# vision-agh/apse_uav

Measured on AMD Instinct MI355X. Metric: 4K UAV frames/sec (whole node), higher is better.
Workload: dtype f32

## Files before the change

### apse_uav_amd/_lib.py

```python
import ctypes as C
import os

import numpy as np

_HERE = os.path.dirname(os.path.abspath(__file__))
_TREE_LIB = os.path.join(_HERE, "libapse_hip.so")
LIB_PATH = os.environ.get("APSE_HIP_LIB") or _TREE_LIB
TOOL_ENTRIES = ("apse_conv2d_ex", "apse_winograd_pack_filter", "apse_winograd_conv2d", "apse_winograd_conv2d_split", "apse_lane_stats", "apse_rpn_select", "apse_box_inference",
                "apse_c4_rpn_select", "apse_rpn_select_train", "apse_rpn_train_proposals_workspace_bytes", "apse_rpn_train_proposals",
                "apse_set_rpn_head", "apse_preprocess_frames_yuv", "apse_yuv_to_bgr", "apse_yuv_matrix_host", "apse_resize_normalize_yuv")

APSE_OK = 0


class ApseError(RuntimeError):
    pass


class Config(C.Structure):
    _fields_ = [
        ("struct_size", C.c_int), ("device", C.c_int), ("max_batch", C.c_int),
        ("frame_h", C.c_int), ("frame_w", C.c_int), ("image_h", C.c_int), ("image_w", C.c_int),
        ("blocks", C.c_int * 4), ("num_classes", C.c_int),
        ("score_thresh", C.c_float), ("box_nms", C.c_float), ("rpn_nms", C.c_float), ("mask_thresh", C.c_float),
        ("rpn_pre_topk", C.c_int), ("rpn_post_topk", C.c_int), ("dets_per_image", C.c_int),
        ("pixel_mean", C.c_float * 3), ("assoc_roi", C.c_int), ("embed_dim", C.c_int), ("assoc_scale", C.c_float),
        ("compute_dtype", C.c_int), ("storage16", C.c_int),
    ]


class ConfigArch(Config):
    _fields_ = [("arch", C.c_int)]


class ConfigLane(ConfigArch):
    _fields_ = [("tail_lane", C.c_int)]


class ResultsLayout(C.Structure):
    _fields_ = [("bytes", C.c_size_t), ("n_max", C.c_int), ("dets_per_image", C.c_int), ("embed_dim", C.c_int),
                ("max_batch", C.c_int)] + [(k, C.c_size_t) for k in (
# ... 30 lines not shown
    "apse_set_resize_tables": ([vp, vp, vp, i, vp, vp, i], i),
    "apse_set_camera": ([vp, C.POINTER(C.c_double), C.POINTER(C.c_double), i, vp, i, i], i),
    "apse_preprocess_frames": ([vp, vp, i, vp], i),
    "apse_preprocess_images": ([vp, vp, i, vp], i),
    "apse_backbone": ([vp, i, vp], i),
    "apse_rpn": ([vp, i, vp], i),
    "apse_rpn_levels": ([vp, i, i, vp], i),
    "apse_box_head": ([vp, i, vp], i),
    "apse_set_detections": ([vp, vp, vp, vp, vp, i, vp], i),
    "apse_mask_tail": ([vp, i, vp], i),
    "apse_embed": ([vp, i, vp], i),
    "apse_forward": ([vp, i, vp], i),
    "apse_results_describe": ([vp, C.POINTER(ResultsLayout)], i),
    "apse_read_results": ([vp, vp, sz, vp], i),
    "apse_read_results_begin": ([vp, vp, sz, vp], i),
    "apse_read_results_end": ([vp, vp], i),
    "apse_lane_stats": ([vp, C.POINTER(C.c_longlong * 4)], i),
    "apse_copy_mask_window": ([vp, i, i, i, i, i, vp, vp], i),
    "apse_copy_mask_windows": ([vp, i, vp, vp, vp, vp, vp], i),
    "apse_host_copy": ([vp, vp, sz, i], i),
    "apse_feature_shape": ([vp, C.c_char_p, C.POINTER(C.c_int * 3)], i),
    "apse_export_feature": ([vp, C.c_char_p, vp, i, vp], i),
    "apse_debug_tensor": ([vp, C.c_char_p, vp, sz, C.POINTER(sz), vp], i),
    "apse_flops": ([vp, i, C.c_double, C.c_double], C.c_double),
    "apse_profile": ([vp, i], i),
    "apse_profile_read": ([vp, C.POINTER(C.c_double * 42), i], i),
    "apse_conv_packed_elems": ([C.POINTER(ConvDesc)], sz),
    "apse_conv_pack_weight": ([C.POINTER(ConvDesc), vp, i, vp, vp], i),
    "apse_conv2d": ([C.POINTER(ConvDesc), vp, vp, vp, vp, vp, vp, sz, vp], i),
    "apse_conv2d_ex": ([C.POINTER(ConvDesc), vp, vp, vp, vp, vp, vp, sz, vp, i, i, i, vp], i),
    "apse_winograd_pack_filter": ([vp, i, i, vp], i),
    "apse_winograd_conv2d": ([C.POINTER(ConvDesc), vp, vp, vp, vp, vp], i),
    "apse_winograd_conv2d_split": ([C.POINTER(ConvDesc), vp, vp, vp, vp, vp, C.c_size_t, i, vp], i),
    "apse_maxpool3x3s2": ([vp, vp, i, i, i, i, vp], i),
    "apse_maxpool3x3s2_typed": ([vp, vp, i, i, i, i, i, vp], i),
    "apse_roi_align": ([C.POINTER(vp), C.POINTER(i), C.POINTER(i), vp, i, i, i, vp, vp], i),
    "apse_roi_align_typed": ([C.POINTER(vp), C.POINTER(i), C.POINTER(i), vp, i, i, i, i, vp, vp], i),
    "apse_roi_pool": ([vp, i, i, vp, vp, i, i, f, vp, vp], i),
    "apse_roi_features": ([vp, i, vp, vp, i, i, vp, vp], i),
    "apse_nms_rank": ([vp, vp, vp, i, i, i, i, f, i, vp, vp, vp, vp, vp], i),
    "apse_rpn_select": ([C.POINTER(vp), C.POINTER(i), C.POINTER(i), i, i, i, i, i, i, f, i, vp, vp, vp, vp, vp, vp, vp, vp, vp], i),
    "apse_box_inference": ([vp, i, i, vp, vp, i, i, i, i, f, f, i, i] + [vp] * 16, i),
    "apse_c4_rpn_select": ([vp, i, i, i, i, i, i, i, f, vp, vp, vp, vp, vp, vp, vp, vp], i),
    "apse_mask_centroid_dense": ([vp, i, i, C.POINTER(C.c_int * 3), vp], i),
    "apse_mask_closest_dense": ([vp, i, i, f, f, C.POINTER(C.c_int * 2), vp], i),
    "apse_l2_normalize": ([vp, vp, i, i, vp], i),
    "apse_sqdist": ([vp, vp, i, i, i, vp, vp], i),
    "apse_undistort_gamma": ([vp, vp, i, i, i, C.POINTER(C.c_double), C.POINTER(C.c_double), i, vp, i, i, vp], i),
    "apse_lab_tables_host": ([vp, vp, C.c_size_t], C.c_size_t),
    "apse_replay_create": ([i, i, f, i], vp),
    "apse_replay_destroy": ([vp], None),
    "apse_replay_step": ([vp, i, i, vp, vp, vp, C.c_char_p, i, vp], i),
    "apse_replay_packed": ([vp, vp, C.c_longlong, i, i, i, vp, C.c_longlong], C.c_longlong),
    "apse_replay_max_id": ([vp], i),
    "apse_replay_next_id": ([vp], i),
    "apse_render_workspace_bytes": ([i, i, i], sz),
    "apse_render_instances": ([vp, vp, i, i, i, i, vp, i, vp, sz, vp, i, vp, sz, vp], i),
    "apse_render_pack_mask": ([vp, i, i, vp, vp], i),
    "apse_render_font_host": ([vp, sz], sz),
    "apse_mots_split_workspace_bytes": ([], sz),
    "apse_mots_split_idmap": ([vp, i, i, i, vp, sz, vp, vp, vp, vp, sz, vp], i),
    "apse_mots_rle_to_bits": ([vp, vp, i, i, i, vp, vp], i),
    "apse_mots_overlaps": ([vp, i, vp, i, vp, i, vp, vp], i),
    "apse_mots_shift_overlaps": ([vp, i, vp, i, i, i, vp, vp], i),
    "apse_mots_render_idmap": ([vp, vp, i, i, i, vp, vp], i),
    "apse_mots_crop_overlaps": ([vp, vp, i, i, i, vp, sz, vp, vp, vp], i),
# ... 106 lines not shown
```

### apse_uav_amd/csrc/conv_igemm.hip

```cpp
#include "apse_common.h"
#include <type_traits>

typedef _Float16 f16x8 __attribute__((ext_vector_type(8)));
__device__ __forceinline__ f32x16 apse_mfma16(bf16x8 a, bf16x8 b, f32x16 c) { return __builtin_amdgcn_mfma_f32_32x32x16_bf16(a, b, c, 0, 0, 0); }
__device__ __forceinline__ f32x16 apse_mfma16(f16x8 a, f16x8 b, f32x16 c) { return __builtin_amdgcn_mfma_f32_32x32x16_f16(a, b, c, 0, 0, 0); }

template <int WM, int WN, int TM, int TN, int KS, int XT, int WK, int PR = 0>
__global__ __launch_bounds__(64 * WM * WN * WK) void conv_igemm_f32(const ConvParams p) {
    static_assert(PR == 0 || XT == 0, "16-bit operands use the descriptor path only");
    constexpr bool DESC = XT != 1;
    constexpr int EPS = PR ? 64 : 32;
    constexpr int ESH = PR ? 1 : 2;
    constexpr int EPSLOT = 16 >> ESH;
    constexpr int NT = 64 * WM * WN * WK;
    constexpr int BM = WM * TM * 32;
    constexpr int BN = WN * TN * 32;
    constexpr int SR = NT / 8;
    constexpr int AP = BM / SR;
    constexpr int BP = BN / SR;
    static_assert(AP >= 1 && BP >= 1 && KS % WK == 0 && (DESC || WK == 1), "unsupported shape");
    constexpr int LDC = BN + 4;
    constexpr bool DP = DESC && (TM * TN <= 2 || (PR != 0 && WM * WN == 8 && APSE_DP16));
    constexpr int NSET = DP ? 2 : 1;
    constexpr int STORE_AT = 4 * KS - 2;
    extern __shared__ __attribute__((aligned(16))) char smem[];
    float* As = reinterpret_cast<float*>(smem);
    float* Bs = As + 2 * KS * BM * 32;
    float* Cs = reinterpret_cast<float*>(smem);

    const int tid = threadIdx.x;
    const int lane = tid & 63;
    const int wave = tid >> 6;
    const int kg = wave / (WM * WN);
    const int wm = (wave % (WM * WN)) / WN, wn = wave % WN;
    const int fr = lane & 31, fh = lane >> 5;
    const int srow = tid >> 3, slot = tid & 7;

    int M = p.M;
    if (p.m_count) {
        int lim = (*p.m_count) * p.m_per_item;
        M = lim < M ? lim : M;
    }
    const int tiles_n = (p.Cout + BN - 1) / BN;
    const int tiles_m = (M + BM - 1) / BM;
    const int nwg = tiles_m * tiles_n;
    const int z = blockIdx.y;
    const int steps_per_row = p.KWCp / EPS;
    const int steps_total = PR ? p.KH * steps_per_row : p.steps_total;
    const int steps_big = (steps_total + KS - 1) / KS;
    const int per = (steps_big + p.splitk - 1) / p.splitk;
    const int s_begin = z * per;
    const int s_end = (s_begin + per < steps_big) ? s_begin + per : steps_big;
    const int ohw = p.OH * p.OW;
    const size_t w_row = (size_t)p.KH * p.KWCp;
    const bool direct = (p.splitk == 1);
    __amdgpu_buffer_rsrc_t xrsrc;
    if constexpr (DESC)
        xrsrc = __builtin_amdgcn_make_buffer_rsrc(const_cast<float*>(p.x), 0, (int)((((unsigned)(p.B * p.H * p.W) << p.cin_log2)) << (XT >= 2 ? 1 : ESH)), 0x00020000);

    bool warm_pending = p.next_w && z == 0;
    for (int wg = blockIdx.x; wg < nwg; wg += gridDim.x) {
        const int bid = apse_xcd_remap(wg, nwg);
        const int tile_m = bid / tiles_n, tile_n = bid - tile_m * tiles_n;
        const int m0 = tile_m * BM, n0 = tile_n * BN;

        int a_iy0[AP], a_ix0[AP], a_pix[AP], a_base[AP];
#pragma unroll
        for (int i = 0; i < AP; ++i) {
            const int m = m0 + srow + SR * i;
            if (m < M) {
                const int b = m / ohw;
                const int rem = m - b * ohw;
                const int oy = rem / p.OW;
                const int ox = rem - oy * p.OW;
                a_iy0[i] = oy * p.stride - p.pad;
                a_ix0[i] = ox * p.stride - p.pad;
                a_pix[i] = b * p.H * p.W;
            } else {
                a_iy0[i] = -(1 << 28);
                a_ix0[i] = 0;
                a_pix[i] = 0;
            }
            a_base[i] = (a_pix[i] + a_iy0[i] * p.W + a_ix0[i]) << p.cin_log2;
        }

        f32x4 ra[NSET][KS][AP], rb[NSET][KS][BP];
        int ld_r, ld_q;
        {
            const int ss0 = s_begin * KS;
            ld_r = ss0 / steps_per_row;
            ld_q = ss0 - ld_r * steps_per_row;
        }
        const char* wrow[BP];
#pragma unroll
        for (int i = 0; i < BP; ++i)
            wrow[i] = (PR ? reinterpret_cast<const char*>(p.w16) : reinterpret_cast<const char*>(p.w)) +
                      ((((size_t)(n0 + srow + SR * i) * w_row) + (size_t)(slot * EPSLOT)) << ESH);
        int cur_r = 0, cur_ry = 0, cur_q = 0, cur_rowoff = 0, cur_woff = 0, cur_dpx = 0;
        auto fetch_piece = [&](int set, int u, int j) {
            if (j == 0) {
                const bool live = ld_r < p.KH;
                cur_r = live ? ld_r : p.KH - 1;
                cur_ry = live ? ld_r : (1 << 28);
                cur_q = ld_q * EPS + slot * EPSLOT;
                cur_dpx = cur_q >> p.cin_log2;
                cur_rowoff = ((cur_r * p.W) << p.cin_log2) + cur_q;
                cur_woff = (cur_r * p.KWCp + ld_q * EPS) << ESH;
                ++ld_q;
                if (ld_q == steps_per_row) { ld_q = 0; ++ld_r; }
            }
            if (j < AP) {
                const int iy = a_iy0[j] + cur_ry;
                const int px = a_ix0[j] + cur_dpx;
                const int okm = -(int)(((unsigned)iy < (unsigned)p.H) & ((unsigned)px < (unsigned)p.W));
                if constexpr (XT >= 2) {
                    const unsigned off = (((unsigned)(a_base[j] + cur_rowoff) << 1) & (unsigned)okm) | (0xfffffff0u & ~(unsigned)okm);
                    const auto raw = __builtin_amdgcn_raw_buffer_load_b64(xrsrc, (int)off, 0, 0);
                    ra[set][u][j] = f32x4{__uint_as_float(raw[0]), __uint_as_float(raw[1]), 0.f, 0.f};
                } else {
                    const unsigned off = (((unsigned)(a_base[j] + cur_rowoff) << ESH) & (unsigned)okm) | (0xfffffff0u & ~(unsigned)okm);
                    ra[set][u][j] = __builtin_bit_cast(f32x4, __builtin_amdgcn_raw_buffer_load_b128(xrsrc, (int)off, 0, 0));
                }
            } else {
                rb[set][u][j - AP] = *reinterpret_cast<const f32x4*>(wrow[j - AP] + cur_woff);
            }
        };
        auto store_piece = [&](int set, int buf, int u, int j) {
            if (j < AP) {
                const int row = srow + SR * j;
                const int ps = slot ^ ((row >> 1) & 7);
                f32x4 v = ra[set][u][j];
                if constexpr (XT == 2) {
// ... 472 lines not shown
            if (p.res_st == 1) return __uint_as_float((uint32_t)reinterpret_cast<const uint16_t*>(p.res)[idx] << 16);
            return (float)reinterpret_cast<const _Float16*>(p.res)[idx];
        };
        size_t dst;
        if (p.out_mode == 0) {
            if (p.res_mode == 1) {
                val += ld1((size_t)m * p.Cout + n);
            } else if (p.res_mode == 2) {
                const int b = m / ohw;
                const int rem = m - b * ohw;
                const int oy = rem / p.OW, ox = rem - oy * p.OW;
                const int hw2 = (p.OH >> 1) * (p.OW >> 1);
                val += ld1(((size_t)b * hw2 + (oy >> 1) * (p.OW >> 1) + (ox >> 1)) * p.Cout + n);
            }
            dst = (size_t)m * p.y_ld + p.y_coff + n;
        } else {
            const int b = m / ohw;
            const int rem = m - b * ohw;
            const int oy = rem / p.OW, ox = rem - oy * p.OW;
            const int dy = g >> 1, dx = g & 1;
            dst = (((size_t)b * 2 * p.OH + 2 * oy + dy) * (2 * p.OW) + 2 * ox + dx) * p.cdec + co;
        }
        if (p.relu) val = apse_relu(val);
        apse_st1(p.y, dst, val, p.y_st);
    }
}

void apse_launch_splitk_reduce4(const ConvParams& p, hipStream_t s) {
    int blocks = (int)(((size_t)p.M * p.Cout / 4 + 255) / 256);
    if (blocks > 4096) blocks = 4096;
    hipLaunchKernelGGL(conv_splitk_reduce4, dim3(blocks), dim3(256), 0, s, p);
}

template <int WM, int WN, int TM, int TN, int KS, int XT, int WK = 1, int PR = 0>
static int launch_cfg_x(const ConvParams& p, hipStream_t s, hipEvent_t ev0, hipEvent_t ev1) {
    constexpr int BM = WM * TM * 32, BN = WN * TN * 32;
    const int tiles = ((p.M + BM - 1) / BM) * ((p.Cout + BN - 1) / BN);
    const size_t lds_stage = (size_t)2 * KS * (BM + BN) * 32 * sizeof(float), lds_c = (size_t)WK * BM * (BN + 4) * sizeof(float) + 16;
    const size_t lds = lds_stage > lds_c ? lds_stage : lds_c;
    static bool attr_done = false;
    if (!attr_done) {
        hipFuncSetAttribute(reinterpret_cast<const void*>(&conv_igemm_f32<WM, WN, TM, TN, KS, XT, WK, PR>),
                            hipFuncAttributeMaxDynamicSharedMemorySize, (int)lds);
        attr_done = true;
    }
    int grid_x = tiles;
    if (p.m_count) {
        int want = 1024;
        if (p.m_hint > 0) {
            want = 2 * ((p.m_hint + BM - 1) / BM) * ((p.Cout + BN - 1) / BN);
            if (want < 64) want = 64;
            if (want > 1024) want = 1024;
        }
        if (grid_x > want) grid_x = want;
    }
    if (ev0) hipEventRecord(ev0, s);
    hipLaunchKernelGGL((conv_igemm_f32<WM, WN, TM, TN, KS, XT, WK, PR>), dim3(grid_x, p.splitk), dim3(64 * WM * WN * WK), lds, s, p);
    if (ev1) hipEventRecord(ev1, s);
    if (p.splitk > 1 && !p.tile_cnt) {
        const size_t total = (size_t)p.M * p.Cout;
        const bool vec4 = p.out_mode == 0 && (p.res_mode == 0 || p.res_mode == 1) && ((p.Cout | p.y_ld | p.y_coff) & 3) == 0 && total < 0x7fffffffull;
        int blocks = (int)(((vec4 ? total / 4 : total) + 255) / 256);
        if (blocks > 4096) blocks = 4096;
        if (vec4) hipLaunchKernelGGL(conv_splitk_reduce4, dim3(blocks), dim3(256), 0, s, p);
        else hipLaunchKernelGGL(conv_splitk_reduce, dim3(blocks), dim3(256), 0, s, p);
    }
    return hipGetLastError() == hipSuccess ? APSE_OK : APSE_E_HIP;
}

static bool descriptor_ok(const ConvParams& p) { return p.x_st == 0 && (((size_t)p.B * p.H * p.W) << p.cin_log2) * 4 < 0xfffffff0ull; }

template <int WM, int WN, int TM, int TN, int KS>
static int launch_cfg(const ConvParams& p, hipStream_t s, hipEvent_t ev0, hipEvent_t ev1) {
    return descriptor_ok(p) ? launch_cfg_x<WM, WN, TM, TN, KS, 0>(p, s, ev0, ev1) : launch_cfg_x<WM, WN, TM, TN, KS, 1>(p, s, ev0, ev1);
}
template <int WM, int WN, int TM, int TN, int KS, int KSF>
static int launch_cfg_k2(const ConvParams& p, hipStream_t s, hipEvent_t ev0, hipEvent_t ev1) {
    return descriptor_ok(p) ? launch_cfg_x<WM, WN, TM, TN, KS, 0, 2>(p, s, ev0, ev1) : launch_cfg_x<WM, WN, TM, TN, KSF, 1>(p, s, ev0, ev1);
}

static int fast16_shape(const ConvParams& p, int cfg) {
    const bool fast16 = (p.prec == 1 || p.prec == 2) && p.w16 && p.x_st == p.prec && (p.KWCp & 63) == 0 && p.cin_log2 >= 3 &&
                        ((((size_t)p.B * p.H * p.W) << p.cin_log2) * 2 < 0xfffffff0ull) && !p.tile_cnt;
    if (!fast16) return -1;
    int c16 = (cfg == 4 || cfg == 5 || cfg == 2) ? 1 : (cfg == 7 ? 6 : cfg);
    if (c16 == 0 && p.steps_total >= 16 && ((p.M + 255) / 256) * ((p.Cout + 127) / 128) >= 250) c16 = 8;
    return c16;
}

int apse_conv_effective_cfg(const ConvParams& p, int cfg) {
    if (cfg == APSE_CFG_STREAM) return (!p.no_stream && apse_conv1x1_stream_ok(p)) ? APSE_CFG_STREAM : -1;
    if (cfg == APSE_CFG_GLDS) return apse_conv_glds16_ok(p) ? APSE_CFG_GLDS : -1;
    if (cfg == APSE_CFG_SKINNY) return apse_conv_skinny_ok(p) ? APSE_CFG_SKINNY : -1;
    if (!p.no_stream && apse_conv_skinny_ok(p)) return APSE_CFG_SKINNY;
    if (!p.no_stream && apse_conv1x1_stream_ok(p)) return APSE_CFG_STREAM;
    if (!p.no_stream && apse_conv_glds16_ok(p)) {
        const int c16 = fast16_shape(p, cfg);
        if (c16 == 8) return APSE_CFG_GLDS;
        const int t128 = ((p.M + 127) / 128) * ((p.Cout + 127) / 128);
        if ((c16 == 0 || c16 == 3) && p.steps_total >= 16 && t128 >= 200 && t128 <= 320 && apse_conv_glds16_small(p)) return APSE_CFG_GLDS;
    }
    return cfg;
}

int apse_launch_conv(const ConvParams& p, int cfg, hipStream_t s, hipEvent_t ev0, hipEvent_t ev1) {
    if (p.M <= 0 || p.Cout <= 0 || p.steps_total <= 0) return APSE_E_INVALID;
    if (p.res_mode != 0 && (p.Cout & 3) != 0) return APSE_E_INVALID;
    const int eff = apse_conv_effective_cfg(p, cfg);
    if (eff < 0) return APSE_E_INVALID;
    if (eff == APSE_CFG_STREAM) return apse_launch_conv1x1_stream(p, s, ev0, ev1);
    if (eff == APSE_CFG_GLDS) return apse_launch_conv_glds16(p, s, ev0, ev1);
    if (eff == APSE_CFG_SKINNY) return apse_launch_conv_skinny(p, s, ev0, ev1);
    if (p.prec == 1 || p.prec == 2) {
        const int c16 = fast16_shape(p, cfg);
        if (c16 >= 0) {
            int rc = APSE_E_INVALID;
            if (p.prec == 1) {
                if (c16 == 0) rc = launch_cfg_x<2, 2, 2, 2, 1, 0, 1, 1>(p, s, ev0, ev1);
                else if (c16 == 1) rc = launch_cfg_x<2, 2, 1, 1, 2, 0, 1, 1>(p, s, ev0, ev1);
                else if (c16 == 3) rc = launch_cfg_x<4, 1, 1, 2, 1, 0, 1, 1>(p, s, ev0, ev1);
                else if (c16 == 6) rc = launch_cfg_x<2, 2, 1, 1, 2, 0, 2, 1>(p, s, ev0, ev1);
                else if (c16 == 8) rc = launch_cfg_x<4, 2, 2, 2, 1, 0, 1, 1>(p, s, ev0, ev1);
            } else {
                if (c16 == 0) rc = launch_cfg_x<2, 2, 2, 2, 1, 0, 1, 2>(p, s, ev0, ev1);
                else if (c16 == 1) rc = launch_cfg_x<2, 2, 1, 1, 2, 0, 1, 2>(p, s, ev0, ev1);
                else if (c16 == 3) rc = launch_cfg_x<4, 1, 1, 2, 1, 0, 1, 2>(p, s, ev0, ev1);
                else if (c16 == 6) rc = launch_cfg_x<2, 2, 1, 1, 2, 0, 2, 2>(p, s, ev0, ev1);
                else if (c16 == 8) rc = launch_cfg_x<4, 2, 2, 2, 1, 0, 1, 2>(p, s, ev0, ev1);
            }
            return rc;
        }
        return APSE_E_INVALID;
    }
    switch (cfg) {
        case 0: return launch_cfg<2, 2, 2, 2, 1>(p, s, ev0, ev1);
        case 1: return launch_cfg<2, 2, 1, 1, 2>(p, s, ev0, ev1);
        case 2: {
            const bool small = (((size_t)p.B * p.H * p.W) << p.cin_log2) * 4 < 0xfffffff0ull;
            if (small && p.x_st == 1 && p.cin_log2 >= 2) return launch_cfg_x<4, 1, 1, 1, 2, 2>(p, s, ev0, ev1);
            if (small && p.x_st == 2 && p.cin_log2 >= 2) return launch_cfg_x<4, 1, 1, 1, 2, 3>(p, s, ev0, ev1);
            return launch_cfg<4, 1, 1, 1, 2>(p, s, ev0, ev1);
        }
        case 3: return launch_cfg<4, 1, 1, 2, 1>(p, s, ev0, ev1);
        case 4: return launch_cfg<2, 2, 1, 1, 1>(p, s, ev0, ev1);
        case 5: return launch_cfg<4, 1, 1, 1, 1>(p, s, ev0, ev1);
        case 6: return launch_cfg_k2<2, 2, 1, 1, 2, 2>(p, s, ev0, ev1);
        case 7: return launch_cfg_k2<2, 2, 1, 1, 4, 2>(p, s, ev0, ev1);
        case 8: return launch_cfg<2, 2, 2, 2, 1>(p, s, ev0, ev1);
        default: return APSE_E_INVALID;
    }
}

int apse_conv_pick_cfg(int M, int Cout, int steps, int* splitk) {
    *splitk = 1;
    auto tiles = [&](int bm, int bn) { return ((M + bm - 1) / bm) * ((Cout + bn - 1) / bn); };
    auto split_for = [&](int t, int min_steps_per_split) {
        int sk = (512 + t / 2) / t;
        if (sk > steps / min_steps_per_split) sk = steps / min_steps_per_split;
        if (sk > 64) sk = 64;
        return sk < 1 ? 1 : sk;
    };
    if (Cout <= 32) {
        const int t = tiles(128, 32);
        if (t < 32 && steps >= 16) {
            int sk = 64 / t;
            if (sk > steps / 4) sk = steps / 4;
            if (sk > 8) sk = 8;
            *splitk = sk < 1 ? 1 : sk;
        }
        return 2;
    }
    if (Cout <= 64) return tiles(128, 64) >= 192 ? 3 : 1;
    const int t128 = tiles(128, 128);
    if (t128 >= 224) {
        if (t128 < 384 && tiles(128, 64) >= 384) return 3;
        return 0;
    }
    if (t128 >= 32 && steps >= 256) {
        *splitk = split_for(t128, 8);
// ... 15 lines not shown
```

### apse_uav_amd/csrc/conv_winograd.hip

```cpp
#include "apse_common.h"

namespace {
constexpr int WT = 64;
constexpr int WN = 64;
constexpr int KC = 8;
constexpr int NTHR = 512;
constexpr int G_U = 1, G_ROWS = 2, G_V = 3;
constexpr int SLICE_F = 16 * WT * KC;
constexpr size_t WINO_LDS = (size_t)2 * 2 * SLICE_F * sizeof(float);
static_assert(WN == WT, "V and U slices share one size");
static_assert((size_t)16 * WT * 32 * sizeof(float) <= WINO_LDS, "epilogue chunk must fit the staging LDS");
}

template <int WTR, int WTC, bool SPLIT>
__global__ __launch_bounds__(NTHR) void conv_winograd_f32(const ConvParams p) {
    static_assert(WTR * WTC == WT, "64 tiles per block");
    extern __shared__ __attribute__((aligned(16))) char smem[];
    float* Vs = reinterpret_cast<float*>(smem);
    float* Us = Vs + 2 * SLICE_F;
    float* Cs = reinterpret_cast<float*>(smem);

    const int tid = threadIdx.x;
    const int lane = tid & 63, wave = __builtin_amdgcn_readfirstlane(tid >> 6);
    const int fr = lane & 31, fh = lane >> 5;

    const int tiles_y = (p.OH + 2 * WTR - 1) / (2 * WTR), tiles_x = (p.OW + 2 * WTC - 1) / (2 * WTC);
    const int nblk = p.Cout / WN;
    const int nwg = p.B * tiles_y * tiles_x * nblk;
    const int bid = apse_xcd_remap(blockIdx.x, nwg);
    const int nb = bid % nblk;
    int rest = bid / nblk;
    const int bx = rest % tiles_x; rest /= tiles_x;
    const int by = rest % tiles_y;
// ... 11 lines not shown
    const int cg = tid & 1, t = (tid >> 1) & (WT - 1), ti = wave >> 1;
    const int ra = ti == 0 ? 0 : (ti == 2 ? 2 : 1);
    const int rb = ti == 0 ? 2 : (ti == 1 ? 2 : (ti == 2 ? 1 : 3));
    const float sgn = ti == 1 ? 1.f : -1.f;
    const int iy_a = oy0 + 2 * (t / WTC) - 1 + ra, iy_b = oy0 + 2 * (t / WTC) - 1 + rb;
    const int ix0 = ox0 + 2 * (t % WTC) - 1;
    const __amdgpu_buffer_rsrc_t xrsrc =
        __builtin_amdgcn_make_buffer_rsrc(const_cast<float*>(p.x), 0, (int)((((unsigned)(p.B * p.H * p.W)) << p.cin_log2) * 4u), 0x00020000);
    const __amdgpu_buffer_rsrc_t xnone = __builtin_amdgcn_make_buffer_rsrc(const_cast<float*>(p.x), 0, 0, 0x00020000);
    unsigned xoff[2][4];
#pragma unroll
    for (int r = 0; r < 2; ++r) {
        const int iy = r ? iy_b : iy_a;
#pragma unroll
        for (int c = 0; c < 4; ++c) {
            const int ix = ix0 + c;
            const bool in = (unsigned)iy < (unsigned)p.H && (unsigned)ix < (unsigned)p.W;
            xoff[r][c] = in ? ((((unsigned)((b * p.H + iy) * p.W + ix)) << p.cin_log2) + (unsigned)(cg * 4)) * 4u : 0x80000000u;
        }
    }
    const unsigned ustep = (unsigned)(16 * p.Cout * KC * 4);
    const __amdgpu_buffer_rsrc_t ursrc = __builtin_amdgcn_make_buffer_rsrc(
        const_cast<float*>(p.wu), 0, SPLIT ? (int)((unsigned)s_end * ustep) : (int)((((unsigned)(16 * p.Cout)) << p.cin_log2) * 4u), 0x00020000);
    unsigned uoff[4], ulds[4];
#pragma unroll
    for (int k = 0; k < 4; ++k) {
        const int q = tid + NTHR * k;
        const int xi = q >> 7, co = (q >> 1) & 63, h = q & 1;
        uoff[k] = (unsigned)(((xi * p.Cout + n0 + co) * KC + h * 4) * 4);
        ulds[k] = (unsigned)((xi * WN + co) * KC + ((h ^ ((co >> 3) & 1)) * 4));
    }
    const int vlds = (4 * ti * WT + t) * KC + (cg ^ ((t >> 3) & 1)) * 4;

    f32x4 xr[2][4], ur[4];
    auto fetch_u = [&](int s) {
        const unsigned kb = (unsigned)(s_begin + s) * ustep;
#pragma unroll
        for (int k = 0; k < 4; ++k) ur[k] = __builtin_bit_cast(f32x4, __builtin_amdgcn_raw_buffer_load_b128(ursrc, (int)(uoff[k] + kb), 0, 0));
    };
    auto fetch_x = [&](int s) {
        const unsigned kb = (unsigned)((s_begin + s) * KC * 4);
        const __amdgpu_buffer_rsrc_t rs = s < nsteps ? xrsrc : xnone;
#pragma unroll
        for (int r = 0; r < 2; ++r)
#pragma unroll
            for (int c = 0; c < 4; ++c)
                xr[r][c] = __builtin_bit_cast(f32x4, __builtin_amdgcn_raw_buffer_load_b128(rs, (int)(xoff[r][c] + kb), 0, 0));
    };
    auto write_u = [&](int buf) {
#pragma unroll
        for (int k = 0; k < 4; ++k) *reinterpret_cast<f32x4*>(Us + buf * SLICE_F + ulds[k]) = ur[k];
    };
    auto xform_rows = [&]() {
#pragma unroll
        for (int c = 0; c < 4; ++c)
#pragma unroll
            for (int e = 0; e < 4; ++e) xr[0][c][e] = __builtin_fmaf(xr[1][c][e], sgn, xr[0][c][e]);
    };
    auto write_v = [&](int buf) {
        const f32x4 v[4] = {xr[0][0] - xr[0][2], xr[0][1] + xr[0][2], xr[0][2] - xr[0][1], xr[0][1] - xr[0][3]};
#pragma unroll
        for (int j = 0; j < 4; ++j) *reinterpret_cast<f32x4*>(Vs + buf * SLICE_F + vlds + j * WT * KC) = v[j];
    };

    f32x16 acc[2][2][2];
#pragma unroll
    for (int a = 0; a < 2; ++a)
#pragma unroll
        for (int i = 0; i < 2; ++i)
#pragma unroll
            for (int j = 0; j < 2; ++j)
#pragma unroll
                for (int v = 0; v < 16; ++v) acc[a][i][j][v] = 0.f;

    fetch_u(0);
    fetch_x(0);
    write_u(0);
    xform_rows();
    write_v(0);
    __builtin_amdgcn_sched_barrier(0);
    fetch_u(1);
    __builtin_amdgcn_sched_barrier(0);
    fetch_x(1);
    __syncthreads();
    const int fsw = (fh ^ ((fr >> 3) & 1)) * 4;
    const int frag = (2 * wave * WT + fr) * KC + fsw;
    f32x4 af[2][2], bf[2][2];
    auto read_frags = [&](int buf, int a) {
#pragma unroll
        for (int i = 0; i < 2; ++i) af[a][i] = *reinterpret_cast<const f32x4*>(Vs + buf * SLICE_F + frag + (a * WT + 32 * i) * KC);
#pragma unroll
        for (int j = 0; j < 2; ++j) bf[a][j] = *reinterpret_cast<const f32x4*>(Us + buf * SLICE_F + frag + (a * WN + 32 * j) * KC);
    };
    auto mfma_group = [&](int a, int k) {
#pragma unroll
        for (int i = 0; i < 2; ++i)
#pragma unroll
            for (int j = 0; j < 2; ++j)
                acc[a][i][j] = __builtin_amdgcn_mfma_f32_32x32x2f32(af[a][i][k], bf[a][j][k], acc[a][i][j], 0, 0, 0);
    };
    read_frags(0, 0);
    for (int s = 0; s < nsteps; ++s) {
        const int buf = s & 1;
        read_frags(buf, 1);
#pragma unroll
        for (int g = 0; g < 7; ++g) {
            __builtin_amdgcn_sched_barrier(0);
            if (g == G_U) { write_u(buf ^ 1); fetch_u(s + 2); }
            if (g == G_ROWS) xform_rows();
            if (g == G_V) { write_v(buf ^ 1); fetch_x(s + 2); }
            __builtin_amdgcn_sched_barrier(0);
            mfma_group(g >> 2, g & 3);
        }
        __builtin_amdgcn_sched_barrier(0);
        __syncthreads();
        read_frags(buf ^ 1, 0);
        __builtin_amdgcn_sched_barrier(0);
        mfma_group(1, 3);
    }

    const int et = tid >> 3, eg = tid & 7;
    const int oy = oy0 + 2 * (et / WTC), ox = ox0 + 2 * (et % WTC);
    typedef unsigned u32x4_t __attribute__((ext_vector_type(4)));
#pragma unroll
    for (int j = 0; j < 2; ++j) {
#pragma unroll
        for (int a = 0; a < 2; ++a)
#pragma unroll
            for (int i = 0; i < 2; ++i)
#pragma unroll
                for (int v = 0; v < 16; ++v) {
                    const int row = 32 * i + (v & 3) + 8 * (v >> 2) + 4 * fh;
                    Cs[((2 * wave + a) * WT + row) * 32 + fr] = acc[a][i][j][v];
                }
        __syncthreads();
        f32x4 m[16];
#pragma unroll
        for (int k = 0; k < 16; ++k) m[k] = *reinterpret_cast<const f32x4*>(Cs + (k * WT + et) * 32 + eg * 4);
        f32x4 s0[4], s1[4];
#pragma unroll
        for (int c = 0; c < 4; ++c) {
            s0[c] = m[c] + m[4 + c] + m[8 + c];
            s1[c] = m[4 + c] - m[8 + c] - m[12 + c];
        }
        const int co = n0 + 32 * j + 4 * eg;
        if constexpr (SPLIT) {
            float* slab = p.ws + (size_t)blockIdx.y * p.M * p.Cout;
#pragma unroll
            for (int dy = 0; dy < 2; ++dy)
#pragma unroll
                for (int dx = 0; dx < 2; ++dx) {
// ... 61 lines not shown
```

### include/apse_hip.h

```cpp
#ifndef APSE_HIP_H
#define APSE_HIP_H
#include <stddef.h>
#include <stdint.h>
#ifdef __cplusplus
extern "C" {
#endif

#define APSE_OK 0
#define APSE_E_INVALID (-1)
#define APSE_E_HIP (-2)
#define APSE_E_NOMEM (-3)
#define APSE_E_STATE (-4)
#define APSE_E_MISSING (-5)

typedef struct apse_ctx apse_ctx;

#define APSE_MAX_CLASSES 80
#define APSE_C4_MAX_PRE_TOPK 6000
#define APSE_C4_MAX_BATCH 2
#define APSE_MAX_FRAME_W 49152
#define APSE_MAX_FRAME_H 32768
typedef struct apse_config {
    int struct_size;
    int device;
// ... 72 lines not shown
int apse_read_results(apse_ctx* ctx, void* host_dst, size_t bytes, void* stream);
int apse_read_results_begin(apse_ctx* ctx, void* host_dst, size_t bytes, void* stream);
int apse_read_results_end(apse_ctx* ctx, void* host_dst);
int apse_lane_stats(apse_ctx* ctx, long long* out4);
int apse_copy_mask_window(apse_ctx* ctx, int det, int x0, int y0, int x1, int y1, uint64_t* dst_dev, void* stream);
int apse_copy_mask_windows(apse_ctx* ctx, int n, const int* dets_host, const int* rects_host, uint64_t* dst_dev,
                           const long long* dst_word_offsets_host, void* stream);
int apse_feature_shape(apse_ctx* ctx, const char* name, int* chw3);
int apse_export_feature(apse_ctx* ctx, const char* name, float* dst_nchw_dev, int batch, void* stream);
int apse_debug_tensor(apse_ctx* ctx, const char* name, void* dst_dev, size_t max_bytes, size_t* bytes, void* stream);
double apse_flops(apse_ctx* ctx, int batch, double proposals, double detections);

int apse_profile(apse_ctx* ctx, int enable);
int apse_profile_read(apse_ctx* ctx, double* out42, int reset);

typedef struct apse_conv_desc {
    int B, H, W, Cin;
    int Cout, KH, KW, stride, pad;
    int relu;
    int res_mode;
    int cfg;
    int splitk;
    int prec;
    int fuse_reduce;
    int x_st, res_st, y_st;
} apse_conv_desc;
size_t apse_conv_packed_elems(const apse_conv_desc* d);
int apse_conv_pack_weight(const apse_conv_desc* d, const float* w_oihw, int cin_real, const float* scale, float* packed);
int apse_conv2d(const apse_conv_desc* d, const float* x_dev, const float* w_packed_dev, const float* bias_dev,
                const float* res_dev, float* y_dev, float* ws_dev, size_t ws_bytes, void* stream);
int apse_conv2d_ex(const apse_conv_desc* d, const void* x_dev, const float* w_packed_dev, const float* bias_dev, const void* res_dev,
                   void* y_dev, float* ws_dev, size_t ws_bytes, const int* count_dev, int hint_items, int y_ld, int deconv,
                   void* stream);
int apse_winograd_pack_filter(const float* w_oihw, int Cout, int Cin, float* packed);
int apse_winograd_conv2d(const apse_conv_desc* d, const float* x_dev, const float* wu_dev, const float* bias_dev, float* y_dev,
                         void* stream);
int apse_winograd_conv2d_split(const apse_conv_desc* d, const float* x_dev, const float* wu_dev, const float* bias_dev, float* y_dev,
                               float* ws_dev, size_t ws_bytes, int geometry, void* stream);
int apse_maxpool3x3s2(const float* x_dev, float* y_dev, int B, int H, int W, int C, void* stream);
int apse_maxpool3x3s2_typed(const void* x_dev, void* y_dev, int B, int H, int W, int C, int storage, void* stream);
int apse_roi_align(const float* const* feats_dev, const int* hs, const int* ws, const float* rois_dev, int n, int per_img,
                   int out_size, float* out_dev, void* stream);
int apse_roi_align_typed(const void* const* feats_dev, const int* hs, const int* ws, const float* rois_dev, int n, int per_img,
                         int out_size, int storage, void* out_dev, void* stream);
int apse_roi_pool(const float* feat_dev, int H, int W, const float* rois_dev, const int* roi_img_dev, int n, int out_size,
                  float scale, float* out_dev, void* stream);
int apse_nms_rank(const float* boxes_dev, const float* scores_dev, const int* valid_dev, int n, int cat_div, int cat_mod,
                  int ncat, float thr, int topk, float* out_boxes_dev, float* out_scores_dev, int* out_index_dev,
                  int* out_count_dev, void* stream);
int apse_rpn_select(const float* const* heads_dev, const int* H, const int* W, int head_ld, int B, int image_h, int image_w,
                    int pre_topk, int post_topk, float nms_thr, int level_mask, unsigned long long* keys_dev, float* dec_boxes_dev,
                    float* dec_scores_dev, int* dec_valid_dev, float* props_dev, float* prop_scores_dev, int* prop_entry_dev,
                    int* prop_count_dev, void* stream);
int apse_box_inference(const float* pred_dev, int ld, int K, const float* props_dev, const int* prop_cnt_dev, int P, int B,
                       int image_h, int image_w, float score_thresh, float nms_thr, int dets_per_image, int wide,
                       float* probs_dev, float* cand_boxes_dev, float* cand_scores_dev, int* cand_valid_dev, float* det_boxes_dev,
                       float* det_scores_dev, int* det_entry_dev, int* det_cnt_dev, float* pk_boxes_dev, float* pk_scores_dev,
                       int* pk_cls_dev, int* pk_img_dev, int* pk_roi_dev, int* pk_total_dev, int* pk_offset_dev, void* stream);
int apse_c4_rpn_select(const float* head_dev, int H, int W, int B, int image_h, int image_w, int pre, int post, float nms_thr,
                       float* dec_boxes_dev, float* dec_scores_dev, int* dec_valid_dev, float* props_dev, float* prop_scores_dev,
                       int* prop_entry_dev, int* prop_count_dev, void* stream);
int apse_mask_centroid_dense(const uint8_t* mask_dev, int H, int W, int* out_xy_mass_host3, void* stream);
int apse_mask_closest_dense(const uint8_t* mask_dev, int H, int W, float px, float py, int* out_xy_host2, void* stream);
int apse_l2_normalize(const float* x_dev, float* y_dev, int n, int D, void* stream);
int apse_sqdist(const float* a_dev, const float* b_dev, int O, int N, int D, float* out_dev, void* stream);
int apse_undistort_gamma(const uint8_t* src_dev, uint8_t* dst_dev, int B, int H, int W, const double* mtx3x3_host,
// ... 219 lines not shown
```

Baseline: 208.2.

## Add pointwise 1x1 conv address path and unroll Winograd loop by buffer parity

Adds a specialized implicit-GEMM kernel variant for 1x1 stride-free convolutions that precomputes per-thread byte offsets and issues buffer loads with a scalar step offset, for both activations and weights. Out-of-range steps are masked by building a zero-size descriptor instead of clamping row indices. This removes the per-step KH/KW address recomputation for pointwise layers. Separately, the Winograd kernel moves the step offset into the scalar soffset field, guards filter loads past the last step, and unrolls the main loop by two so the LDS buffer index is a compile-time constant. A launch counter is exported for testing, and an env var can disable the new path.

```diff
diff --git a/apse_uav_amd/_lib.py b/apse_uav_amd/_lib.py
--- a/apse_uav_amd/_lib.py
+++ b/apse_uav_amd/_lib.py
@@ -6,7 +6,7 @@
 _HERE = os.path.dirname(os.path.abspath(__file__))
 _TREE_LIB = os.path.join(_HERE, "libapse_hip.so")
 LIB_PATH = os.environ.get("APSE_HIP_LIB") or _TREE_LIB
-TOOL_ENTRIES = ("apse_conv2d_ex", "apse_winograd_pack_filter", "apse_winograd_conv2d", "apse_winograd_conv2d_split", "apse_lane_stats", "apse_rpn_select", "apse_box_inference",
+TOOL_ENTRIES = ("apse_conv2d_ex", "apse_winograd_pack_filter", "apse_winograd_conv2d", "apse_winograd_conv2d_split", "apse_conv_pointwise_launches", "apse_lane_stats", "apse_rpn_select", "apse_box_inference",
                 "apse_c4_rpn_select", "apse_rpn_select_train", "apse_rpn_train_proposals_workspace_bytes", "apse_rpn_train_proposals",
                 "apse_set_rpn_head", "apse_preprocess_frames_yuv", "apse_yuv_to_bgr", "apse_yuv_matrix_host", "apse_resize_normalize_yuv")
 
@@ -103,6 +103,7 @@
     "apse_winograd_pack_filter": ([vp, i, i, vp], i),
     "apse_winograd_conv2d": ([C.POINTER(ConvDesc), vp, vp, vp, vp, vp], i),
     "apse_winograd_conv2d_split": ([C.POINTER(ConvDesc), vp, vp, vp, vp, vp, C.c_size_t, i, vp], i),
+    "apse_conv_pointwise_launches": ([], C.c_uint),
     "apse_maxpool3x3s2": ([vp, vp, i, i, i, i, vp], i),
     "apse_maxpool3x3s2_typed": ([vp, vp, i, i, i, i, i, vp], i),
     "apse_roi_align": ([C.POINTER(vp), C.POINTER(i), C.POINTER(i), vp, i, i, i, vp, vp], i),
diff --git a/apse_uav_amd/csrc/conv_igemm.hip b/apse_uav_amd/csrc/conv_igemm.hip
--- a/apse_uav_amd/csrc/conv_igemm.hip
+++ b/apse_uav_amd/csrc/conv_igemm.hip
@@ -1,13 +1,18 @@
 #include "apse_common.h"
+#include <atomic>
 #include <type_traits>
 
 typedef _Float16 f16x8 __attribute__((ext_vector_type(8)));
 __device__ __forceinline__ f32x16 apse_mfma16(bf16x8 a, bf16x8 b, f32x16 c) { return __builtin_amdgcn_mfma_f32_32x32x16_bf16(a, b, c, 0, 0, 0); }
 __device__ __forceinline__ f32x16 apse_mfma16(f16x8 a, f16x8 b, f32x16 c) { return __builtin_amdgcn_mfma_f32_32x32x16_f16(a, b, c, 0, 0, 0); }
 
-template <int WM, int WN, int TM, int TN, int KS, int XT, int WK, int PR = 0>
+struct apse_pointwise {};
+template <int WM, int WN, int TM, int TN, int KS, int XT, int WK, int PR = 0, typename... FORM>
 __global__ __launch_bounds__(64 * WM * WN * WK) void conv_igemm_f32(const ConvParams p) {
+    static_assert(sizeof...(FORM) == 0 || (sizeof...(FORM) == 1 && (std::is_same<FORM, apse_pointwise>::value && ...)), "FORM is nothing or apse_pointwise");
+    constexpr bool PW = sizeof...(FORM) != 0;
     static_assert(PR == 0 || XT == 0, "16-bit operands use the descriptor path only");
+    static_assert(!PW || XT == 0, "the pointwise address form exists for the plain descriptor path only");
     constexpr bool DESC = XT != 1;
     constexpr int EPS = PR ? 64 : 32;
     constexpr int ESH = PR ? 1 : 2;
@@ -55,8 +60,13 @@
     const size_t w_row = (size_t)p.KH * p.KWCp;
     const bool direct = (p.splitk == 1);
     __amdgpu_buffer_rsrc_t xrsrc;
+    const unsigned xbytes = (((unsigned)(p.B * p.H * p.W) << p.cin_log2)) << (XT >= 2 ? 1 : ESH);
     if constexpr (DESC)
-        xrsrc = __builtin_amdgcn_make_buffer_rsrc(const_cast<float*>(p.x), 0, (int)((((unsigned)(p.B * p.H * p.W) << p.cin_log2)) << (XT >= 2 ? 1 : ESH)), 0x00020000);
+        xrsrc = __builtin_amdgcn_make_buffer_rsrc(const_cast<float*>(p.x), 0, (int)xbytes, 0x00020000);
+    __amdgpu_buffer_rsrc_t wrsrc;
+    if constexpr (PW)
+        wrsrc = __builtin_amdgcn_make_buffer_rsrc(PR ? const_cast<void*>(reinterpret_cast<const void*>(p.w16)) : const_cast<void*>(reinterpret_cast<const void*>(p.w)), 0,
+                                                  (int)(((unsigned)((p.Cout + 127) & ~127) * (unsigned)w_row) << ESH), 0x00020000);
 
     bool warm_pending = p.next_w && z == 0;
     for (int wg = blockIdx.x; wg < nwg; wg += gridDim.x) {
@@ -97,7 +107,34 @@
             wrow[i] = (PR ? reinterpret_cast<const char*>(p.w16) : reinterpret_cast<const char*>(p.w)) +
                       ((((size_t)(n0 + srow + SR * i) * w_row) + (size_t)(slot * EPSLOT)) << ESH);
         int cur_r = 0, cur_ry = 0, cur_q = 0, cur_rowoff = 0, cur_woff = 0, cur_dpx = 0;
+        unsigned pw_a[AP], pw_w[BP];
+        int pw_s = s_begin * KS, pw_soff = 0;
+        unsigned pw_xbytes = 0;
+        if constexpr (PW) {
+#pragma unroll
+            for (int i = 0; i < AP; ++i) {
+                const bool in = ((unsigned)a_iy0[i] < (unsigned)p.H) & ((unsigned)a_ix0[i] < (unsigned)p.W);
+                pw_a[i] = in ? ((unsigned)(a_base[i] + slot * EPSLOT) << ESH) : 0xfffffff0u;
+            }
+#pragma unroll
+            for (int i = 0; i < BP; ++i) pw_w[i] = ((unsigned)(n0 + srow + SR * i) * (unsigned)w_row + (unsigned)(slot * EPSLOT)) << ESH;
+        }
         auto fetch_piece = [&](int set, int u, int j) {
+            if constexpr (PW) {
+                if (j == 0) {
+                    const bool live = pw_s < steps_total;
+                    pw_soff = live ? pw_s * 128 : 0;
+                    pw_xbytes = live ? xbytes : 0u;
+                    ++pw_s;
+                }
+                if (j < AP) {
+                    const __amdgpu_buffer_rsrc_t xs = __builtin_amdgcn_make_buffer_rsrc(const_cast<float*>(p.x), 0, (int)pw_xbytes, 0x00020000);
+                    ra[set][u][j] = __builtin_bit_cast(f32x4, __builtin_amdgcn_raw_buffer_load_b128(xs, (int)pw_a[j], pw_soff, 0));
+                } else {
+                    rb[set][u][j - AP] = __builtin_bit_cast(f32x4, __builtin_amdgcn_raw_buffer_load_b128(wrsrc, (int)pw_w[j - AP], pw_soff, 0));
+                }
+                return;
+            }
             if (j == 0) {
                 const bool live = ld_r < p.KH;
                 cur_r = live ? ld_r : p.KH - 1;
@@ -636,7 +673,10 @@
     hipLaunchKernelGGL(conv_splitk_reduce4, dim3(blocks), dim3(256), 0, s, p);
 }
 
-template <int WM, int WN, int TM, int TN, int KS, int XT, int WK = 1, int PR = 0>
+static std::atomic<unsigned> g_pointwise_launches{0};
+extern "C" unsigned apse_conv_pointwise_launches(void) { return g_pointwise_launches.load(std::memory_order_relaxed); }
+
+template <int WM, int WN, int TM, int TN, int KS, int XT, int WK = 1, int PR = 0, bool PW = false>
 static int launch_cfg_x(const ConvParams& p, hipStream_t s, hipEvent_t ev0, hipEvent_t ev1) {
     constexpr int BM = WM * TM * 32, BN = WN * TN * 32;
     const int tiles = ((p.M + BM - 1) / BM) * ((p.Cout + BN - 1) / BN);
@@ -644,8 +684,12 @@
     const size_t lds = lds_stage > lds_c ? lds_stage : lds_c;
     static bool attr_done = false;
     if (!attr_done) {
-        hipFuncSetAttribute(reinterpret_cast<const void*>(&conv_igemm_f32<WM, WN, TM, TN, KS, XT, WK, PR>),
-                            hipFuncAttributeMaxDynamicSharedMemorySize, (int)lds);
+        if constexpr (PW)
+            hipFuncSetAttribute(reinterpret_cast<const void*>(&conv_igemm_f32<WM, WN, TM, TN, KS, XT, WK, PR, apse_pointwise>),
+                                hipFuncAttributeMaxDynamicSharedMemorySize, (int)lds);
+        else
+            hipFuncSetAttribute(reinterpret_cast<const void*>(&conv_igemm_f32<WM, WN, TM, TN, KS, XT, WK, PR>),
+                                hipFuncAttributeMaxDynamicSharedMemorySize, (int)lds);
         attr_done = true;
     }
     int grid_x = tiles;
@@ -659,7 +703,12 @@
         if (grid_x > want) grid_x = want;
     }
     if (ev0) hipEventRecord(ev0, s);
-    hipLaunchKernelGGL((conv_igemm_f32<WM, WN, TM, TN, KS, XT, WK, PR>), dim3(grid_x, p.splitk), dim3(64 * WM * WN * WK), lds, s, p);
+    if constexpr (PW) {
+        hipLaunchKernelGGL((conv_igemm_f32<WM, WN, TM, TN, KS, XT, WK, PR, apse_pointwise>), dim3(grid_x, p.splitk), dim3(64 * WM * WN * WK), lds, s, p);
+        g_pointwise_launches.fetch_add(1, std::memory_order_relaxed);
+    } else {
+        hipLaunchKernelGGL((conv_igemm_f32<WM, WN, TM, TN, KS, XT, WK, PR>), dim3(grid_x, p.splitk), dim3(64 * WM * WN * WK), lds, s, p);
+    }
     if (ev1) hipEventRecord(ev1, s);
     if (p.splitk > 1 && !p.tile_cnt) {
         const size_t total = (size_t)p.M * p.Cout;
@@ -674,13 +723,33 @@
 
 static bool descriptor_ok(const ConvParams& p) { return p.x_st == 0 && (((size_t)p.B * p.H * p.W) << p.cin_log2) * 4 < 0xfffffff0ull; }
 
-template <int WM, int WN, int TM, int TN, int KS>
+static bool igemm_addr_on() {
+    static const bool on = [] { const char* e = getenv("APSE_IGEMM_ADDR"); return !(e && e[0] == '0'); }();
+    return on;
+}
+static bool pointwise_ok(const ConvParams& p) {
+    return igemm_addr_on() && p.KH == 1 && p.KW == 1 && p.pad == 0 && p.KWCp == (1 << p.cin_log2) &&
+           (size_t)((p.Cout + 127) & ~127) * (size_t)p.KWCp * 4 < 0xfffffff0ull;
+}
+
+template <int WM, int WN, int TM, int TN, int KS, bool PWF = false>
 static int launch_cfg(const ConvParams& p, hipStream_t s, hipEvent_t ev0, hipEvent_t ev1) {
-    return descriptor_ok(p) ? launch_cfg_x<WM, WN, TM, TN, KS, 0>(p, s, ev0, ev1) : launch_cfg_x<WM, WN, TM, TN, KS, 1>(p, s, ev0, ev1);
-}
-template <int WM, int WN, int TM, int TN, int KS, int KSF>
+    if (!descriptor_ok(p)) return launch_cfg_x<WM, WN, TM, TN, KS, 1>(p, s, ev0, ev1);
+    if constexpr (PWF)
+        if (pointwise_ok(p)) return launch_cfg_x<WM, WN, TM, TN, KS, 0, 1, 0, true>(p, s, ev0, ev1);
+    return launch_cfg_x<WM, WN, TM, TN, KS, 0>(p, s, ev0, ev1);
+}
+template <int WM, int WN, int TM, int TN, int KS, int KSF, bool PWF = false>
 static int launch_cfg_k2(const ConvParams& p, hipStream_t s, hipEvent_t ev0, hipEvent_t ev1) {
-    return descriptor_ok(p) ? launch_cfg_x<WM, WN, TM, TN, KS, 0, 2>(p, s, ev0, ev1) : launch_cfg_x<WM, WN, TM, TN, KSF, 1>(p, s, ev0, ev1);
+    if (!descriptor_ok(p)) return launch_cfg_x<WM, WN, TM, TN, KSF, 1>(p, s, ev0, ev1);
+    if constexpr (PWF)
+        if (pointwise_ok(p)) return launch_cfg_x<WM, WN, TM, TN, KS, 0, 2, 0, true>(p, s, ev0, ev1);
+    return launch_cfg_x<WM, WN, TM, TN, KS, 0, 2>(p, s, ev0, ev1);
+}
+template <int WM, int WN, int TM, int TN, int KS, int WK, int PR>
+static int launch_cfg16(const ConvParams& p, hipStream_t s, hipEvent_t ev0, hipEvent_t ev1) {
+    if (pointwise_ok(p)) return launch_cfg_x<WM, WN, TM, TN, KS, 0, WK, PR, true>(p, s, ev0, ev1);
+    return launch_cfg_x<WM, WN, TM, TN, KS, 0, WK, PR>(p, s, ev0, ev1);
 }
 
 static int fast16_shape(const ConvParams& p, int cfg) {
@@ -720,16 +789,16 @@
         if (c16 >= 0) {
             int rc = APSE_E_INVALID;
             if (p.prec == 1) {
-                if (c16 == 0) rc = launch_cfg_x<2, 2, 2, 2, 1, 0, 1, 1>(p, s, ev0, ev1);
-                else if (c16 == 1) rc = launch_cfg_x<2, 2, 1, 1, 2, 0, 1, 1>(p, s, ev0, ev1);
-                else if (c16 == 3) rc = launch_cfg_x<4, 1, 1, 2, 1, 0, 1, 1>(p, s, ev0, ev1);
-                else if (c16 == 6) rc = launch_cfg_x<2, 2, 1, 1, 2, 0, 2, 1>(p, s, ev0, ev1);
+                if (c16 == 0) rc = launch_cfg16<2, 2, 2, 2, 1, 1, 1>(p, s, ev0, ev1);
+                else if (c16 == 1) rc = launch_cfg16<2, 2, 1, 1, 2, 1, 1>(p, s, ev0, ev1);
+                else if (c16 == 3) rc = launch_cfg16<4, 1, 1, 2, 1, 1, 1>(p, s, ev0, ev1);
+                else if (c16 == 6) rc = launch_cfg16<2, 2, 1, 1, 2, 2, 1>(p, s, ev0, ev1);
                 else if (c16 == 8) rc = launch_cfg_x<4, 2, 2, 2, 1, 0, 1, 1>(p, s, ev0, ev1);
             } else {
-                if (c16 == 0) rc = launch_cfg_x<2, 2, 2, 2, 1, 0, 1, 2>(p, s, ev0, ev1);
-                else if (c16 == 1) rc = launch_cfg_x<2, 2, 1, 1, 2, 0, 1, 2>(p, s, ev0, ev1);
-                else if (c16 == 3) rc = launch_cfg_x<4, 1, 1, 2, 1, 0, 1, 2>(p, s, ev0, ev1);
-                else if (c16 == 6) rc = launch_cfg_x<2, 2, 1, 1, 2, 0, 2, 2>(p, s, ev0, ev1);
+                if (c16 == 0) rc = launch_cfg16<2, 2, 2, 2, 1, 1, 2>(p, s, ev0, ev1);
+                else if (c16 == 1) rc = launch_cfg16<2, 2, 1, 1, 2, 1, 2>(p, s, ev0, ev1);
+                else if (c16 == 3) rc = launch_cfg16<4, 1, 1, 2, 1, 1, 2>(p, s, ev0, ev1);
+                else if (c16 == 6) rc = launch_cfg16<2, 2, 1, 1, 2, 2, 2>(p, s, ev0, ev1);
                 else if (c16 == 8) rc = launch_cfg_x<4, 2, 2, 2, 1, 0, 1, 2>(p, s, ev0, ev1);
             }
             return rc;
@@ -737,18 +806,18 @@
         return APSE_E_INVALID;
     }
     switch (cfg) {
-        case 0: return launch_cfg<2, 2, 2, 2, 1>(p, s, ev0, ev1);
-        case 1: return launch_cfg<2, 2, 1, 1, 2>(p, s, ev0, ev1);
+        case 0: return launch_cfg<2, 2, 2, 2, 1, true>(p, s, ev0, ev1);
+        case 1: return launch_cfg<2, 2, 1, 1, 2, true>(p, s, ev0, ev1);
         case 2: {
             const bool small = (((size_t)p.B * p.H * p.W) << p.cin_log2) * 4 < 0xfffffff0ull;
             if (small && p.x_st == 1 && p.cin_log2 >= 2) return launch_cfg_x<4, 1, 1, 1, 2, 2>(p, s, ev0, ev1);
             if (small && p.x_st == 2 && p.cin_log2 >= 2) return launch_cfg_x<4, 1, 1, 1, 2, 3>(p, s, ev0, ev1);
             return launch_cfg<4, 1, 1, 1, 2>(p, s, ev0, ev1);
         }
-        case 3: return launch_cfg<4, 1, 1, 2, 1>(p, s, ev0, ev1);
+        case 3: return launch_cfg<4, 1, 1, 2, 1, true>(p, s, ev0, ev1);
         case 4: return launch_cfg<2, 2, 1, 1, 1>(p, s, ev0, ev1);
         case 5: return launch_cfg<4, 1, 1, 1, 1>(p, s, ev0, ev1);
-        case 6: return launch_cfg_k2<2, 2, 1, 1, 2, 2>(p, s, ev0, ev1);
+        case 6: return launch_cfg_k2<2, 2, 1, 1, 2, 2, true>(p, s, ev0, ev1);
         case 7: return launch_cfg_k2<2, 2, 1, 1, 4, 2>(p, s, ev0, ev1);
         case 8: return launch_cfg<2, 2, 2, 2, 1>(p, s, ev0, ev1);
         default: return APSE_E_INVALID;
diff --git a/apse_uav_amd/csrc/conv_winograd.hip b/apse_uav_amd/csrc/conv_winograd.hip
--- a/apse_uav_amd/csrc/conv_winograd.hip
+++ b/apse_uav_amd/csrc/conv_winograd.hip
@@ -1,4 +1,5 @@
 #include "apse_common.h"
+#include <type_traits>
 
 namespace {
 constexpr int WT = 64;
@@ -76,20 +77,22 @@
     }
     const int vlds = (4 * ti * WT + t) * KC + (cg ^ ((t >> 3) & 1)) * 4;
 
+    const __amdgpu_buffer_rsrc_t unone = __builtin_amdgcn_make_buffer_rsrc(const_cast<float*>(p.wu), 0, 0, 0x00020000);
     f32x4 xr[2][4], ur[4];
     auto fetch_u = [&](int s) {
-        const unsigned kb = (unsigned)(s_begin + s) * ustep;
-#pragma unroll
-        for (int k = 0; k < 4; ++k) ur[k] = __builtin_bit_cast(f32x4, __builtin_amdgcn_raw_buffer_load_b128(ursrc, (int)(uoff[k] + kb), 0, 0));
+        const int kb = (int)((unsigned)(s_begin + s) * ustep);
+        const __amdgpu_buffer_rsrc_t rs = s < nsteps ? ursrc : unone;
+#pragma unroll
+        for (int k = 0; k < 4; ++k) ur[k] = __builtin_bit_cast(f32x4, __builtin_amdgcn_raw_buffer_load_b128(rs, (int)uoff[k], kb, 0));
     };
     auto fetch_x = [&](int s) {
-        const unsigned kb = (unsigned)((s_begin + s) * KC * 4);
+        const int kb = (s_begin + s) * KC * 4;
         const __amdgpu_buffer_rsrc_t rs = s < nsteps ? xrsrc : xnone;
 #pragma unroll
         for (int r = 0; r < 2; ++r)
 #pragma unroll
             for (int c = 0; c < 4; ++c)
-                xr[r][c] = __builtin_bit_cast(f32x4, __builtin_amdgcn_raw_buffer_load_b128(rs, (int)(xoff[r][c] + kb), 0, 0));
+                xr[r][c] = __builtin_bit_cast(f32x4, __builtin_amdgcn_raw_buffer_load_b128(rs, (int)xoff[r][c], kb, 0));
     };
     auto write_u = [&](int buf) {
 #pragma unroll
@@ -144,8 +147,8 @@
                 acc[a][i][j] = __builtin_amdgcn_mfma_f32_32x32x2f32(af[a][i][k], bf[a][j][k], acc[a][i][j], 0, 0, 0);
     };
     read_frags(0, 0);
-    for (int s = 0; s < nsteps; ++s) {
-        const int buf = s & 1;
+    auto slice = [&](auto BUF, int s) {
+        constexpr int buf = decltype(BUF)::value;
         read_frags(buf, 1);
 #pragma unroll
         for (int g = 0; g < 7; ++g) {
@@ -161,6 +164,10 @@
         read_frags(buf ^ 1, 0);
         __builtin_amdgcn_sched_barrier(0);
         mfma_group(1, 3);
+    };
+    for (int s = 0; s < nsteps; s += 2) {
+        slice(std::integral_constant<int, 0>{}, s);
+        if (s + 1 < nsteps) slice(std::integral_constant<int, 1>{}, s + 1);
     }
 
     const int et = tid >> 3, eg = tid & 7;
diff --git a/include/apse_hip.h b/include/apse_hip.h
--- a/include/apse_hip.h
+++ b/include/apse_hip.h
@@ -128,6 +128,7 @@
 int apse_conv2d_ex(const apse_conv_desc* d, const void* x_dev, const float* w_packed_dev, const float* bias_dev, const void* res_dev,
                    void* y_dev, float* ws_dev, size_t ws_bytes, const int* count_dev, int hint_items, int y_ld, int deconv,
                    void* stream);
+unsigned apse_conv_pointwise_launches(void);
 int apse_winograd_pack_filter(const float* w_oihw, int Cout, int Cin, float* packed);
 int apse_winograd_conv2d(const apse_conv_desc* d, const float* x_dev, const float* wu_dev, const float* bias_dev, float* y_dev,
                          void* stream);
```

Measured after the change: 214.5, median of 6. +3.0%, better.
